# tinganchen/AlignQ

Hardware: AMD Instinct MI355X
Metric: images/sec (train step, CDF+ADMM) ResNet-20 8-bit (higher is better)
Workload: dtype f32; 1 GPU; resnet20 CIFAR-shape 3x32x32, 8W/8A CDF+ADMM full train step (cdf_alignment_admm/resnet-20-cifar-10), batch 128/GPU, HIP-graph replay, batch-norm folded into the site kernels, channels-last tensors, all Conv2d_Q convolutions on alignq_conv*_nhwc (exact-product bf16 MFMA); global_batch=128, parallelism=dp1

## Files before the change

alignq_amd/csrc/conv_kernels.hip:

```cpp
#include <hip/hip_runtime.h>
#include <stdint.h>
#include <stdlib.h>

#include "../../include/alignq.h"
#include "site_internal.h"
#include "wgrad_reduce_body.h"

namespace {

using namespace alignq_wgr;

typedef __bf16 bf16x8 __attribute__((ext_vector_type(8)));
typedef __bf16 bf16x4 __attribute__((ext_vector_type(4)));
typedef float f32x4 __attribute__((ext_vector_type(4)));
typedef short s16x4 __attribute__((ext_vector_type(4)));

__device__ __forceinline__ s16x4 tr_read(const __bf16* p) {
  return __builtin_amdgcn_ds_read_tr16_b64_v4i16((__attribute__((address_space(3))) s16x4*)(p));
}
__device__ __forceinline__ bf16x8 join8(s16x4 a, s16x4 b) {
  typedef short s16x8 __attribute__((ext_vector_type(8)));
  s16x8 v = {a[0], a[1], a[2], a[3], b[0], b[1], b[2], b[3]};
  return __builtin_bit_cast(bf16x8, v);
}


template <int xb>
__device__ __forceinline__ f32x4 fetch_act4(const float* __restrict__ x, int64_t off) {
  if constexpr (xb == 0) return *reinterpret_cast<const f32x4*>(x + off);
  if constexpr (xb == 2) {
    const s16x4 b = *reinterpret_cast<const s16x4*>(reinterpret_cast<const short*>(x) + off);
    return (f32x4){(float)b[0], (float)b[1], (float)b[2], (float)b[3]};
  }
  const char4 b = *reinterpret_cast<const char4*>(reinterpret_cast<const signed char*>(x) + off);
  return (f32x4){(float)b.x, (float)b.y, (float)b.z, (float)b.w};
}

struct BnLazy {
  const float* z;
  const float* ab;
  const float* save;
  const float* ktot;
  const float* part = nullptr;
  int n_tiles = 0, tile_f = 0;
  double inv_n = 1.0;
  float* dgamma = nullptr;
  float* dbeta = nullptr;
};

template <int C>
__device__ __forceinline__ void bn_totals_lds(const BnLazy& t, float* __restrict__ kt, bool publish) {
  static_assert(256 % C == 0, "thread -> (channel, group)");
  __shared__ double red[256][2];
  constexpr int G = 256 / C;
  const int tid = threadIdx.x;
  const int cp = C < t.tile_f ? C : t.tile_f;
  const int cyc = C / cp, cnt = t.n_tiles / cyc;
  const int c = tid % C, grp = tid / C;
// ... 597 lines not shown

template <int CIN, int COUT, int WDI, int KS, int PT>
__global__ __launch_bounds__(256) void dgrad_s2_kernel(const float* __restrict__ dy, const float* __restrict__ w,
                                                       float* __restrict__ dx, int H, int total_rows, float nlev,
                                                       const float* __restrict__ add, BnLazy lazy) {
  __shared__ __attribute__((aligned(16))) __bf16 lds[DgradS2Lds<CIN, COUT, WDI, KS, PT, false>::kBf16];
  dgrad_s2_body<CIN, COUT, WDI, KS, PT, false>(dy, w, dx, H, total_rows, nlev, add, lazy, lds, blockIdx.x);
}

template <int CIN, int COUT, int WDI, int KS, int PT>
int launch_dgrad_s2(const float* dy, const float* w, float* dx, int B, int H, float nlev, const float* add, BnLazy lazy,
                    hipStream_t st) {
  constexpr int TR = PT / WDI;
  static_assert(TR % 2 == 0, "even number of input rows per tile");
  if (H % TR) return ALIGNQ_EUNSUPPORTED;
  const int total_rows = B * H;
  hipLaunchKernelGGL((dgrad_s2_kernel<CIN, COUT, WDI, KS, PT>), total_rows / TR, 256, 0, st, dy, w, dx, H, total_rows, nlev,
                     add, lazy);
  hipError_t e = hipGetLastError();
  return e == hipSuccess ? 0 : (int)e;
}

constexpr int kStemPT = 128;
__device__ __forceinline__ void stem_stage(const float* __restrict__ x, int H, int row0, __bf16* Chi, __bf16* Cmi, __bf16* Clo) {
  const int tid = threadIdx.x;
  const int pix = tid >> 1, half = tid & 1;
  const int r = pix / 32, c = pix % 32;
  const int grow = row0 + r;
  const int ih = grow % H;
  float v[16];
#pragma unroll
  for (int j = 0; j < 16; j++) {
    const int k = 16 * half + j;
    const int tap = k / 3, ci = k % 3;
    const int ky = tap / 3, kx = tap % 3;
    const int yy = ih + ky - 1, xx = c + kx - 1;
    const bool ok = k < 27 && yy >= 0 && yy < H && xx >= 0 && xx < 32;
    v[j] = x[ok ? ((int64_t)(grow + ky - 1) * 32 + xx) * 3 + ci : 0];
    if (!ok) v[j] = 0.f;
  }
  bf16x8 h[2], m[2], l[2];
#pragma unroll
  for (int j = 0; j < 16; j++) {
    const __bf16 hi = (__bf16)v[j];
    const float r1 = v[j] - (float)hi;
    const __bf16 mi = (__bf16)r1;
    h[j >> 3][j & 7] = hi; m[j >> 3][j & 7] = mi; l[j >> 3][j & 7] = (__bf16)(r1 - (float)mi);
  }
  const int o = pix * 32 + 16 * half;
  *reinterpret_cast<bf16x8*>(Chi + o) = h[0]; *reinterpret_cast<bf16x8*>(Chi + o + 8) = h[1];
  *reinterpret_cast<bf16x8*>(Cmi + o) = m[0]; *reinterpret_cast<bf16x8*>(Cmi + o + 8) = m[1];
  *reinterpret_cast<bf16x8*>(Clo + o) = l[0]; *reinterpret_cast<bf16x8*>(Clo + o + 8) = l[1];
}

__global__ __launch_bounds__(256) void stem_fwd_kernel(const float* __restrict__ x, const float* __restrict__ w,
                                                       float* __restrict__ y, int H, int total_rows, float nlev,
                                                       float* __restrict__ bn_part) {
  __shared__ __attribute__((aligned(16))) __bf16 lds[3 * kStemPT * 32];
  __bf16* Chi = lds;
  __bf16* Cmi = lds + kStemPT * 32;
  __bf16* Clo = lds + 2 * kStemPT * 32;
  const int tid = threadIdx.x, lane = tid & 63, wv = tid >> 6;
  const int row0 = blockIdx.x * 4;
  stem_stage(x, H, row0, Chi, Cmi, Clo);
  const int m = lane & 15, q = lane >> 4;
  bf16x8 ab;
#pragma unroll
  for (int j = 0; j < 8; j++) {
    const int k = 8 * q + j;
    ab[j] = (__bf16)rintf((k < 27 ? w[m * 27 + k] : 0.f) * nlev);
  }
  __syncthreads();
  float bs[4] = {0.f, 0.f, 0.f, 0.f}, bq[4] = {0.f, 0.f, 0.f, 0.f};
  for (int g = wv; g < kStemPT / 16; g += 4) {
    const int p = g * 16 + (lane & 15);
// ... 18 lines not shown
      ROW_SHR_ADD(bs[e], 0x111); ROW_SHR_ADD(bs[e], 0x112); ROW_SHR_ADD(bs[e], 0x114); ROW_SHR_ADD(bs[e], 0x118);
      ROW_SHR_ADD(bq[e], 0x111); ROW_SHR_ADD(bq[e], 0x112); ROW_SHR_ADD(bq[e], 0x114); ROW_SHR_ADD(bq[e], 0x118);
    }
#undef ROW_SHR_ADD
    __syncthreads();
    if ((lane & 15) == 15) {
#pragma unroll
      for (int e = 0; e < 4; e++) {
        red[(wv * 16 + 4 * q + e) * 2] = bs[e];
        red[(wv * 16 + 4 * q + e) * 2 + 1] = bq[e];
      }
    }
    __syncthreads();
    if (tid < 16) {
      float s0 = 0.f, s1 = 0.f;
#pragma unroll
      for (int w2 = 0; w2 < 4; w2++) { s0 += red[(w2 * 16 + tid) * 2]; s1 += red[(w2 * 16 + tid) * 2 + 1]; }
      bn_part[((int64_t)tid * gridDim.x + blockIdx.x) * 2] = s0;
      bn_part[((int64_t)tid * gridDim.x + blockIdx.x) * 2 + 1] = s1;
    }
  }
}

__global__ __launch_bounds__(256) void stem_wgrad_kernel(const float* __restrict__ x, const float* __restrict__ dy,
                                                         float* __restrict__ slabs, int H, int n_tiles, BnLazy lazy) {
  __shared__ __attribute__((aligned(16))) __bf16 lds[3 * kStemPT * 32 + 3 * kStemPT * 16];
  __bf16* Ci[3] = {lds, lds + kStemPT * 32, lds + 2 * kStemPT * 32};
  __bf16* Di[3] = {lds + 3 * kStemPT * 32, lds + 3 * kStemPT * 32 + kStemPT * 16, lds + 3 * kStemPT * 32 + 2 * kStemPT * 16};
  const int tid = threadIdx.x, lane = tid & 63, wv = tid >> 6;
  const int g = lane >> 4, q = (lane & 15) >> 2, pcol = 4 * (lane & 3);
  f32x4 acc[2] = {{0.f, 0.f, 0.f, 0.f}, {0.f, 0.f, 0.f, 0.f}};
  __shared__ __attribute__((aligned(16))) float kt[32];
  if (lazy.z && lazy.part) bn_totals_lds<16>(lazy, kt, blockIdx.x == 0);
  for (int tile = blockIdx.x; tile < n_tiles; tile += gridDim.x) {
    const int row0 = tile * 4;
    f32x4 dvr[2], zvr[2];
#pragma unroll
    for (int it = 0; it < 2; it++) {
      const int i = tid + 256 * it;
      const int64_t off = ((int64_t)row0 * 32 + i / 4) * 16 + 4 * (tid % 4);
      dvr[it] = *reinterpret_cast<const f32x4*>(dy + off);
      zvr[it] = lazy.z ? *reinterpret_cast<const f32x4*>(lazy.z + off) : (f32x4){0.f, 0.f, 0.f, 0.f};
    }
    __syncthreads();
    stem_stage(x, H, row0, Ci[0], Ci[1], Ci[2]);
    {
      const int c4 = tid % 4;
      f32x4 la = {0, 0, 0, 0}, lm = la, li = la, lk0 = la, lk1 = la;
      if (lazy.z) {
        la = *reinterpret_cast<const f32x4*>(lazy.ab + 4 * c4);
        lm = *reinterpret_cast<const f32x4*>(lazy.save + 4 * c4);
        li = *reinterpret_cast<const f32x4*>(lazy.save + 16 + 4 * c4);
        const float* kp = lazy.part ? kt : lazy.ktot;
        lk0 = *reinterpret_cast<const f32x4*>(kp + 4 * c4);
        lk1 = *reinterpret_cast<const f32x4*>(kp + 16 + 4 * c4);
      }
#pragma unroll
      for (int it = 0; it < 2; it++) {
        const int i = tid + 256 * it;
        f32x4 dv = dvr[it];
        if (lazy.z) dv = la * (dv - lk0 - (zvr[it] - lm) * li * lk1);
        bf16x4 h4, m4, l4;
#pragma unroll
        for (int e = 0; e < 4; e++) {
          const __bf16 hi = (__bf16)dv[e];
          const float r1 = dv[e] - (float)hi;
          const __bf16 mi = (__bf16)r1;
          h4[e] = hi; m4[e] = mi; l4[e] = (__bf16)(r1 - (float)mi);
        }
        const int o = (i / 4) * 16 + 4 * c4;
        *reinterpret_cast<bf16x4*>(Di[0] + o) = h4;
        *reinterpret_cast<bf16x4*>(Di[1] + o) = m4;
        *reinterpret_cast<bf16x4*>(Di[2] + o) = l4;
      }
    }
    __syncthreads();
    {
      const int p0 = 32 * wv + 8 * g;
      bf16x8 a[3];
#pragma unroll
      for (int t = 0; t < 3; t++) {
        const __bf16* pa = Di[t] + (p0 + q) * 16 + pcol;
        a[t] = join8(tr_read(pa), tr_read(pa + 4 * 16));
      }
#pragma unroll
      for (int blk = 0; blk < 2; blk++) {
        bf16x8 b[3];
#pragma unroll
        for (int t = 0; t < 3; t++) {
          const __bf16* pb = Ci[t] + (p0 + q) * 32 + 16 * blk + pcol;
          b[t] = join8(tr_read(pb), tr_read(pb + 4 * 32));
        }
        f32x4 v = acc[blk];
        v = __builtin_amdgcn_mfma_f32_16x16x32_bf16(a[1], b[1], v, 0, 0, 0);
        v = __builtin_amdgcn_mfma_f32_16x16x32_bf16(a[0], b[2], v, 0, 0, 0);
        v = __builtin_amdgcn_mfma_f32_16x16x32_bf16(a[2], b[0], v, 0, 0, 0);
        v = __builtin_amdgcn_mfma_f32_16x16x32_bf16(a[0], b[1], v, 0, 0, 0);
        v = __builtin_amdgcn_mfma_f32_16x16x32_bf16(a[1], b[0], v, 0, 0, 0);
        v = __builtin_amdgcn_mfma_f32_16x16x32_bf16(a[0], b[0], v, 0, 0, 0);
        acc[blk] = v;
      }
    }
  }
  float* red = reinterpret_cast<float*>(lds);
  __syncthreads();
  if (wv > 0) {
#pragma unroll
    for (int blk = 0; blk < 2; blk++)
#pragma unroll
      for (int e = 0; e < 4; e++) red[(((wv - 1) * 2 + blk) * 4 + e) * 64 + lane] = acc[blk][e];
  }
  __syncthreads();
  if (wv == 0) {
    float* slab = slabs + (int64_t)blockIdx.x * (16 * 27);
#pragma unroll
    for (int blk = 0; blk < 2; blk++) {
#pragma unroll
      for (int e = 0; e < 4; e++) {
        float v = acc[blk][e];
#pragma unroll
        for (int w2 = 0; w2 < 3; w2++) v += red[((w2 * 2 + blk) * 4 + e) * 64 + lane];
        const int k = 16 * blk + (lane & 15), co = 4 * (lane >> 4) + e;
        if (k < 27) slab[co * 27 + k] = v;
// ... 10 lines not shown
  hipLaunchKernelGGL((convgen_fwd_kernel<CIN, COUT, WDI, KS, S, PT>), total_rows / TR, 256, 0, st, x, w, y, H, total_rows,
                     nlev, bn_part);
  hipError_t e = hipGetLastError();
  return e == hipSuccess ? 0 : (int)e;
}

template <int C, int WD, int PT>
int launch(const float* x, const float* w, float* y, int B, int H, int dgrad, float nlev, const float* add, float* bn_part,
           hipStream_t st, int xb = 0, float xlev = 1.0f) {
  constexpr int TR = PT / WD;
  const int total_rows = B * H;
  if (H % TR) return ALIGNQ_EUNSUPPORTED;
  const int grid = total_rows / TR;
  if (dgrad) hipLaunchKernelGGL((conv3x3_nhwc_kernel<C, WD, PT, true, 0>), grid, 256, 0, st, x, w, y, H, total_rows, nlev, add, nullptr, 1.0f);
  else if (xb == 2) hipLaunchKernelGGL((conv3x3_nhwc_kernel<C, WD, PT, false, 2>), grid, 256, 0, st, x, w, y, H, total_rows, nlev, add, bn_part, xlev);
  else if (xb == 1) hipLaunchKernelGGL((conv3x3_nhwc_kernel<C, WD, PT, false, 1>), grid, 256, 0, st, x, w, y, H, total_rows, nlev, add, bn_part, xlev);
  else hipLaunchKernelGGL((conv3x3_nhwc_kernel<C, WD, PT, false, 0>), grid, 256, 0, st, x, w, y, H, total_rows, nlev, add, bn_part, xlev);
  hipError_t e = hipGetLastError();
  return e == hipSuccess ? 0 : (int)e;
}

typedef float f32x16 __attribute__((ext_vector_type(16)));

template <int CIN, int COUT, int WDI, int KS, int S, int PT>
struct WgradGeo {
  static constexpr int WDO = WDI / S, TR = PT / WDO, NT = KS * KS;
  static constexpr int CB = (CIN < COUT ? CIN : COUT) >= 32 ? 32 : 16;
  static constexpr int XROWS = KS == 3 ? TR * S + (S == 1 ? 2 : 1) : TR;
  static constexpr int LW = KS == 3 ? WDI + 2 : WDO;
  static constexpr int XA = XROWS * LW * CB;
  static constexpr int DA = PT * CB;
  static constexpr int kRed = 3 * NT * 4 * 64 * 4;
  static constexpr int kBytes = (3 * (XA + DA) * 2) > kRed ? (3 * (XA + DA) * 2) : kRed;
  static constexpr int kFloats = kBytes / 4;
};
template <int C, int WD, int PT>
struct WgradLds : WgradGeo<C, C, WD, 3, 1, PT> {};

template <int CIN, int COUT, int WDI, int KS, int S, int PT, int XB = 0>
__device__ __forceinline__ void wgrad_body(const float* __restrict__ x, const float* __restrict__ dy,
                                           float* __restrict__ slabs, int H, int n_tiles, float* lds_f, int bx, int gx,
                                           int by, BnLazy lazy = BnLazy{nullptr, nullptr, nullptr, nullptr}, float xlev = 1.0f) {
  constexpr int xb = XB;
  using G = WgradGeo<CIN, COUT, WDI, KS, S, PT>;
  constexpr int WDO = G::WDO, TR = G::TR, NT = G::NT, CB = G::CB, LW = G::LW, XA = G::XA, DA = G::DA, XROWS = G::XROWS;
  constexpr int NBLK = CIN / CB;
  constexpr int NSTEP = PT / 32;
  static_assert(WDO % 8 == 0 && PT % 32 == 0, "a lane group's 8 pixels lie in one output row");
  __bf16* lds = reinterpret_cast<__bf16*>(lds_f);
  __bf16* Xi[3] = {lds, lds + XA, lds + 2 * XA};
  __bf16* Di[3] = {lds + 3 * XA, lds + 3 * XA + DA, lds + 3 * XA + 2 * DA};
  const int tid = threadIdx.x, lane = tid & 63, wv = tid >> 6;
  const int bi = by / NBLK, bj = by % NBLK;
  const int cob = CB == 32 ? (wv >> 1) : 0, cib = CB == 32 ? (wv & 1) : 0;
  const int g = lane >> 4, q = (lane & 15) >> 2, pcol = 4 * (lane & 3);

  f32x4 acc[NT];
#pragma unroll
  for (int t = 0; t < NT; t++) acc[t] = (f32x4){0.f, 0.f, 0.f, 0.f};

  constexpr int C4 = CB / 4;
  constexpr int N4 = XROWS * LW * C4;
  constexpr int M4 = PT * C4;
  constexpr int NIX = (N4 + 255) / 256, NID = (M4 + 255) / 256;
  f32x4 rx[NIX], rd[NID], rz[NID];
  const int per = (n_tiles + gx - 1) / gx;
  const int t_begin = bx * per, t_end = (t_begin + per < n_tiles) ? t_begin + per : n_tiles;
  int nxt = t_begin;
  if (nxt < t_end) {
    const int row0_ = nxt * TR;
    const int img_lo_ = (row0_ / H) * (H * S), img_hi_ = img_lo_ + H * S;
#pragma unroll
    for (int it = 0; it < NIX; it++) {
      const int i = tid + 256 * it;
      const int c4 = i % C4, col = (i / C4) % LW, lr = i / (C4 * LW);
      const int grow = KS == 3 ? row0_ * S - 1 + lr : (row0_ + lr) * S;
      const int gcol = KS == 3 ? col - 1 : col * S;
      const bool ok = i < N4 && gcol >= 0 && gcol < WDI && grow >= img_lo_ && grow < img_hi_;
      const int64_t off = ok ? ((int64_t)grow * WDI + gcol) * CIN + bj * CB + 4 * c4 : 0;
      rx[it] = fetch_act4<XB>(x, off);
      if (!ok) rx[it] = (f32x4){0.f, 0.f, 0.f, 0.f};
    }
#pragma unroll
    for (int it = 0; it < NID; it++) {
      const int i = tid + 256 * it;
      const int64_t off = i < M4 ? ((int64_t)row0_ * WDO + i / C4) * COUT + bi * CB + 4 * (i % C4) : 0;
      rd[it] = *reinterpret_cast<const f32x4*>(dy + off);
      if (lazy.z) rz[it] = *reinterpret_cast<const f32x4*>(lazy.z + off);
    }
  }
  f32x4 la = {0, 0, 0, 0}, lm = la, li = la, lk0 = la, lk1 = la;
  if (lazy.z) {
    const int cq = bi * CB + 4 * (tid % C4);
    la = *reinterpret_cast<const f32x4*>(lazy.ab + cq);
    lm = *reinterpret_cast<const f32x4*>(lazy.save + cq);
    li = *reinterpret_cast<const f32x4*>(lazy.save + COUT + cq);
    if (lazy.part) {
      __shared__ __attribute__((aligned(16))) float kt[2 * COUT];
      bn_totals_lds<COUT>(lazy, kt, false);
      lk0 = *reinterpret_cast<const f32x4*>(kt + cq);
      lk1 = *reinterpret_cast<const f32x4*>(kt + COUT + cq);
    } else {
      lk0 = *reinterpret_cast<const f32x4*>(lazy.ktot + cq);
      lk1 = *reinterpret_cast<const f32x4*>(lazy.ktot + COUT + cq);
    }
  }
  for (int tile = t_begin; tile < t_end; tile++) {
    __syncthreads();
#pragma unroll
    for (int it = 0; it < NIX; it++) {
      const int i = tid + 256 * it;
      if (i < N4) {
        const int c4 = i % C4, col = (i / C4) % LW, lr = i / (C4 * LW);
        bf16x4 h4, m4, l4;
#pragma unroll
        for (int e = 0; e < 4; e++) {
          const float v = rx[it][e];
          const __bf16 hi = (__bf16)v;
          const float r1 = v - (float)hi;
          const __bf16 mi = (__bf16)r1;
          h4[e] = hi; m4[e] = mi; l4[e] = (__bf16)(r1 - (float)mi);
        }
        const int o = (lr * LW + col) * CB + 4 * c4;
        *reinterpret_cast<bf16x4*>(Xi[0] + o) = h4;
        *reinterpret_cast<bf16x4*>(Xi[1] + o) = m4;
        *reinterpret_cast<bf16x4*>(Xi[2] + o) = l4;
      }
    }
#pragma unroll
    for (int it = 0; it < NID; it++) {
      const int i = tid + 256 * it;
      if (i < M4) {
        bf16x4 h4, m4, l4;
        f32x4 dv = rd[it];
        if (lazy.z) dv = la * (dv - lk0 - (rz[it] - lm) * li * lk1);
#pragma unroll
        for (int e = 0; e < 4; e++) {
          const float v = dv[e];
          const __bf16 hi = (__bf16)v;
          const float r1 = v - (float)hi;
          const __bf16 mi = (__bf16)r1;
          h4[e] = hi; m4[e] = mi; l4[e] = (__bf16)(r1 - (float)mi);
        }
        const int o = (i / C4) * CB + 4 * (i % C4);
        *reinterpret_cast<bf16x4*>(Di[0] + o) = h4;
        *reinterpret_cast<bf16x4*>(Di[1] + o) = m4;
        *reinterpret_cast<bf16x4*>(Di[2] + o) = l4;
      }
    }
    __syncthreads();
    nxt = tile + 1;
    if (nxt < t_end) {
      const int row0_ = nxt * TR;
      const int img_lo_ = (row0_ / H) * (H * S), img_hi_ = img_lo_ + H * S;
#pragma unroll
      for (int it = 0; it < NIX; it++) {
        const int i = tid + 256 * it;
        const int c4 = i % C4, col = (i / C4) % LW, lr = i / (C4 * LW);
        const int grow = KS == 3 ? row0_ * S - 1 + lr : (row0_ + lr) * S;
        const int gcol = KS == 3 ? col - 1 : col * S;
        const bool ok = i < N4 && gcol >= 0 && gcol < WDI && grow >= img_lo_ && grow < img_hi_;
        const int64_t off = ok ? ((int64_t)grow * WDI + gcol) * CIN + bj * CB + 4 * c4 : 0;
        rx[it] = fetch_act4<XB>(x, off);
        if (!ok) rx[it] = (f32x4){0.f, 0.f, 0.f, 0.f};
      }
#pragma unroll
      for (int it = 0; it < NID; it++) {
        const int i = tid + 256 * it;
        const int64_t off = i < M4 ? ((int64_t)row0_ * WDO + i / C4) * COUT + bi * CB + 4 * (i % C4) : 0;
        rd[it] = *reinterpret_cast<const f32x4*>(dy + off);
        if (lazy.z) rz[it] = *reinterpret_cast<const f32x4*>(lazy.z + off);
      }
    }
    for (int s = (CB == 16 ? wv : 0); s < NSTEP; s += (CB == 16 ? 4 : 1)) {
      const int p0 = 32 * s + 8 * g;
      const int r = p0 / WDO, c0 = p0 % WDO;
      bf16x8 a[3];
#pragma unroll
      for (int t = 0; t < 3; t++) {
        const __bf16* pa = Di[t] + (p0 + q) * CB + cob * 16 + pcol;
        a[t] = join8(tr_read(pa), tr_read(pa + 4 * CB));
      }
#pragma unroll
      for (int tap = 0; tap < NT; tap++) {
        const int ky = tap / KS, kx = tap % KS;
        bf16x8 b[3];
#pragma unroll
        for (int t = 0; t < 3; t++) {
          const __bf16* pb = Xi[t] + (KS == 3 ? ((r * S + ky) * LW + ((c0 + q) * S + kx)) : (r * LW + c0 + q)) * CB +
                             cib * 16 + pcol;
          b[t] = join8(tr_read(pb), tr_read(pb + 4 * (KS == 3 ? S : 1) * CB));
        }
        f32x4 v = acc[tap];
        v = __builtin_amdgcn_mfma_f32_16x16x32_bf16(a[1], b[1], v, 0, 0, 0);
        if (xb == 0) v = __builtin_amdgcn_mfma_f32_16x16x32_bf16(a[0], b[2], v, 0, 0, 0);
        v = __builtin_amdgcn_mfma_f32_16x16x32_bf16(a[2], b[0], v, 0, 0, 0);
        v = __builtin_amdgcn_mfma_f32_16x16x32_bf16(a[0], b[1], v, 0, 0, 0);
        v = __builtin_amdgcn_mfma_f32_16x16x32_bf16(a[1], b[0], v, 0, 0, 0);
        v = __builtin_amdgcn_mfma_f32_16x16x32_bf16(a[0], b[0], v, 0, 0, 0);
        acc[tap] = v;
      }
    }
  }
  float* slab = slabs + (int64_t)bx * (NT * CIN * COUT);
  if (xb != 0) {
    const float inv = 1.0f / xlev;
#pragma unroll
    for (int t = 0; t < NT; t++) acc[t] = acc[t] * inv;
  }
  if (CB == 16) {
    float* red = lds_f;
    __syncthreads();
    if (wv > 0) {
#pragma unroll
      for (int t = 0; t < NT; t++)
#pragma unroll
        for (int e = 0; e < 4; e++) red[(((wv - 1) * NT + t) * 4 + e) * 64 + lane] = acc[t][e];
    }
    __syncthreads();
    if (wv == 0) {
#pragma unroll
      for (int t = 0; t < NT; t++) {
#pragma unroll
        for (int e = 0; e < 4; e++) {
          float v = acc[t][e];
#pragma unroll
          for (int w2 = 0; w2 < 3; w2++) v += red[((w2 * NT + t) * 4 + e) * 64 + lane];
          __builtin_nontemporal_store(v, &slab[((int64_t)(bi * CB + 4 * (lane >> 4) + e) * NT + t) * CIN + bj * CB + (lane & 15)]);
        }
      }
    }
  } else {
#pragma unroll
    for (int t = 0; t < NT; t++)
#pragma unroll
      for (int e = 0; e < 4; e++)
        __builtin_nontemporal_store(acc[t][e], &slab[((int64_t)(bi * CB + cob * 16 + 4 * (lane >> 4) + e) * NT + t) * CIN + bj * CB + cib * 16 + (lane & 15)]);
  }
}

template <int C, int WD, int PT, int XB = 0>
__device__ __forceinline__ void wgrad3x3_body(const float* __restrict__ x, const float* __restrict__ dy,
                                              float* __restrict__ slabs, int H, int n_tiles, float* lds_f, int bx, int gx,
                                              int by, BnLazy lazy = BnLazy{nullptr, nullptr, nullptr, nullptr}, float xlev = 1.0f) {
  wgrad_body<C, C, WD, 3, 1, PT, XB>(x, dy, slabs, H, n_tiles, lds_f, bx, gx, by, lazy, xlev);
}

template <int CIN, int COUT, int WDI, int KS, int S, int PT>
__global__ __launch_bounds__(256) void wgradgen_kernel(const float* __restrict__ x, const float* __restrict__ dy,
                                                       float* __restrict__ slabs, int H, int n_tiles, BnLazy lazy) {
  __shared__ __attribute__((aligned(16))) float lds[WgradGeo<CIN, COUT, WDI, KS, S, PT>::kFloats];
  wgrad_body<CIN, COUT, WDI, KS, S, PT>(x, dy, slabs, H, n_tiles, lds, blockIdx.x, gridDim.x, blockIdx.y, lazy);
}

template <int C, int WD, int PT, int XB>
__global__ __launch_bounds__(256) void wgrad3x3_nhwc_kernel(const float* __restrict__ x, const float* __restrict__ dy,
                                                            float* __restrict__ slabs, int H, int n_tiles, float xlev) {
  __shared__ __attribute__((aligned(16))) float lds[WgradLds<C, WD, PT>::kFloats];
  wgrad3x3_body<C, WD, PT, XB>(x, dy, slabs, H, n_tiles, lds, blockIdx.x, gridDim.x, blockIdx.y,
                               BnLazy{nullptr, nullptr, nullptr, nullptr}, xlev);
}

template <int C, int WD, int PTD, int PTW, int XB>
__global__ __launch_bounds__(256) void conv3x3_bwd_kernel(const float* __restrict__ x, const float* __restrict__ dy,
                                                          const float* __restrict__ w, float* __restrict__ dx,
                                                          float* __restrict__ slabs, int H, int total_rows, float nlev,
                                                          int n_tiles_w, int splits, int nblk2,
                                                          const float* __restrict__ add, BnLazy lazy, float xlev, int dg_R,
                                                          RedFill fill, int n_dg) {
  constexpr int kBytesD = ConvLds<C, WD, PTD>::kBf16 * 2, kBytesW = WgradLds<C, WD, PTW>::kFloats * 4;
  static_assert(kBytesD >= 4096 || kBytesW >= 4096, "the filler role's 4 KB");
  __shared__ __attribute__((aligned(16))) unsigned char lds[kBytesD > kBytesW ? kBytesD : kBytesW];
  const int n_wg = splits * nblk2;
  if ((int)blockIdx.x < n_wg) {
    wgrad3x3_body<C, WD, PTW, XB>(x, dy, slabs, H, n_tiles_w, reinterpret_cast<float*>(lds), blockIdx.x % splits, splits,
                                  blockIdx.x / splits, lazy, xlev);
  } else if ((int)blockIdx.x >= n_wg + n_dg) {
    const int fb = blockIdx.x - n_wg - n_dg;
    int it = 0;
    while (it + 1 < kFill && fb >= fill.blk0[it + 1]) it++;
    wgrad_reduce_body<256>(fill.slabs[it], fill.n_slabs[it], fill.n_elem[it], fill.dw[it], fb - fill.blk0[it],
                           reinterpret_cast<float*>(lds));
  } else {
    int m = blockIdx.x - n_wg;
    if (dg_R > 0) {
      const int i = (m / (8 * dg_R)) * 8 + (m & 7), r = (m >> 3) % dg_R;
      m = dg_R * i + r;
    }
    conv3x3_body<C, WD, PTD, true>(dy, w, dx, H, total_rows, nlev, reinterpret_cast<__bf16*>(lds), m, add, nullptr, 0, lazy);
  }
}

template <int CIN, int COUT, int WDI, int PTW3, int PTW1, int PTD>
__global__ __launch_bounds__(256) void transition_bwd_kernel(const float* __restrict__ x, const float* __restrict__ dy3,
                                                             const float* __restrict__ dy1, const float* __restrict__ w3,
                                                             const float* __restrict__ w1, float* __restrict__ dx,
                                                             float* __restrict__ slabs3, float* __restrict__ slabs1, int Ho,
                                                             int n_tiles3, int n_tiles1, int splits3, int splits1, int n_d,
                                                             float nlev, const float* __restrict__ add, BnLazy lazy3,
                                                             BnLazy lazy1, int dg_R) {
  using G3 = WgradGeo<CIN, COUT, WDI, 3, 2, PTW3>;
  using G1 = WgradGeo<CIN, COUT, WDI, 1, 2, PTW1>;
  constexpr int NBY = (COUT / G3::CB) * (CIN / G3::CB);
  static_assert(G3::CB == G1::CB, "same channel blocking");
  constexpr int kD = DgradS2Lds<CIN, COUT, WDI, 3, PTD, true>::kBf16 * 2;
  constexpr int kW = G3::kBytes > G1::kBytes ? G3::kBytes : G1::kBytes;
  __shared__ __attribute__((aligned(16))) unsigned char lds[kD > kW ? kD : kW];
  const int n_w3 = splits3 * NBY;
  const int b = blockIdx.x;
  if (b < n_d) {
    int m = b;
    if (dg_R > 0) {
      const int i = (m / (8 * dg_R)) * 8 + (m & 7), r = (m >> 3) % dg_R;
      m = dg_R * i + r;
    }
    dgrad_s2_body<CIN, COUT, WDI, 3, PTD, true>(dy3, w3, dx, 2 * Ho, 0x7fffffff, nlev, add, lazy3,
                                                reinterpret_cast<__bf16*>(lds), m, dy1, w1, lazy1);
  } else if (b < n_d + n_w3) {
    const int c = b - n_d;
    wgrad_body<CIN, COUT, WDI, 3, 2, PTW3>(x, dy3, slabs3, Ho, n_tiles3, reinterpret_cast<float*>(lds), c % splits3, splits3,
                                           c / splits3, lazy3);
  } else {
    const int c = b - n_d - n_w3;
    wgrad_body<CIN, COUT, WDI, 1, 2, PTW1>(x, dy1, slabs1, Ho, n_tiles1, reinterpret_cast<float*>(lds), c % splits1, splits1,
                                           c / splits1, lazy1);
  }
}

__global__ __launch_bounds__(1024) void wgrad_reduce_kernel(const float* __restrict__ slabs, int n_slabs, int n_elem,
                                                            float* __restrict__ dw) {
  __shared__ __attribute__((aligned(16))) float part[4096];
  wgrad_reduce_body(slabs, n_slabs, n_elem, dw, blockIdx.x, part);
}

constexpr int kWgMulti = 32;
struct WgChunk {
  const float* slabs[kWgMulti];
  float* dw[kWgMulti];
  int n_slabs[kWgMulti];
  int n_elem[kWgMulti];
  int blk0[kWgMulti + 1];
};
__global__ __launch_bounds__(1024) void wgrad_reduce_multi_kernel(WgChunk c, int cnt) {
  __shared__ __attribute__((aligned(16))) float part[4096];
// ... 361 lines not shown

int alignq_conv_stem_bn_parts(int B, int H, int W) { return (W == 32 && B >= 1 && H >= 4 && H % 4 == 0) ? B * H / 4 : 0; }
int alignq_conv_stem_nhwc_fwd(const float* x, const float* wt, float* y, int B, int H, int W, int w_bit, float* bn_part,
                              void* stream) {
  if (!x || !wt || !y) return ALIGNQ_EINVAL;
  if (w_bit < 1 || w_bit > 8 || !alignq_conv_stem_bn_parts(B, H, W)) return ALIGNQ_EUNSUPPORTED;
  if (reinterpret_cast<uintptr_t>(y) & 15) return ALIGNQ_EUNSUPPORTED;
  hipLaunchKernelGGL(stem_fwd_kernel, B * H / 4, 256, 0, (hipStream_t)stream, x, wt, y, H, B * H, (float)((1 << w_bit) - 1),
                     bn_part);
  hipError_t e = hipGetLastError();
  return e == hipSuccess ? 0 : (int)e;
}
int alignq_conv_stem_nhwc_wgrad(const float* x, const float* dy, float* dw, void* ws, int B, int H, int W, int* n_slabs_out,
                                const float* bn_z, const float* bn_ab, const float* bn_save, const float* bn_ktot,
                                const float* bn_dx_part, float* bn_dgamma, float* bn_dbeta, void* stream) {
  if (!x || !dy || !ws || (!dw && !n_slabs_out)) return ALIGNQ_EINVAL;
  if (bn_z && (!bn_ab || !bn_save || (!bn_ktot && !bn_dx_part))) return ALIGNQ_EINVAL;
  if (!alignq_conv_stem_bn_parts(B, H, W) || (reinterpret_cast<uintptr_t>(dy) & 15)) return ALIGNQ_EUNSUPPORTED;
  hipStream_t st = (hipStream_t)stream;
  const int n_tiles = B * H / 4;
  const int splits = n_tiles < 256 ? n_tiles : 256;
  BnLazy lazy{bn_z, bn_ab, bn_save, bn_ktot};
  if (int rc = lazy_parts(lazy, bn_dx_part, bn_dgamma, bn_dbeta, B, 16, H * W)) return rc;
  hipLaunchKernelGGL(stem_wgrad_kernel, splits, 256, 0, st, x, dy, (float*)ws, H, n_tiles, lazy);
  hipError_t e = hipGetLastError();
  if (e != hipSuccess) return (int)e;
  if (n_slabs_out) { *n_slabs_out = splits; return 0; }
  hipLaunchKernelGGL(wgrad_reduce_kernel, wgrad_reduce_blocks(splits, 16 * 27), 1024, 0, st, (const float*)ws, splits, 16 * 27, dw);
  e = hipGetLastError();
  return e == hipSuccess ? 0 : (int)e;
}

}
```

Baseline: 126,800 images/sec.

## Prefetch multiple wgrad tiles into registers and drop unused low-part LDS plane

Weight-gradient kernels (stem, 16-channel 3x3 and stride-2 transition) now keep PF tiles of activations and output gradients in flight in registers, issuing the loads for tile t+PF right after parking tile t in LDS. This hides global-load latency behind the MFMA work in the small-channel layers, where each block does little compute per tile. Quantized (int8/int16) inputs are now kept raw in registers, with the zero padding tracked by a bitmask, and the third split plane for X is dropped from LDS because it is never used. The cost is much higher register pressure, which risks lower occupancy or spills.

New measurement: 126,500 images/sec. Within noise of the previous version (-0.3%).

```diff
diff --git a/alignq_amd/csrc/conv_kernels.hip b/alignq_amd/csrc/conv_kernels.hip
--- a/alignq_amd/csrc/conv_kernels.hip
+++ b/alignq_amd/csrc/conv_kernels.hip
@@ -34,6 +34,22 @@
   }
   const char4 b = *reinterpret_cast<const char4*>(reinterpret_cast<const signed char*>(x) + off);
   return (f32x4){(float)b.x, (float)b.y, (float)b.z, (float)b.w};
+}
+
+typedef signed char s8x4 __attribute__((ext_vector_type(4)));
+template <int xb> struct ActRaw { typedef f32x4 T; };
+template <> struct ActRaw<2> { typedef s16x4 T; };
+template <> struct ActRaw<1> { typedef s8x4 T; };
+template <int xb>
+__device__ __forceinline__ typename ActRaw<xb>::T fetch_act_raw(const float* __restrict__ x, int64_t off) {
+  if constexpr (xb == 0) return *reinterpret_cast<const f32x4*>(x + off);
+  if constexpr (xb == 2) return *reinterpret_cast<const s16x4*>(reinterpret_cast<const short*>(x) + off);
+  if constexpr (xb == 1) return *reinterpret_cast<const s8x4*>(reinterpret_cast<const signed char*>(x) + off);
+}
+template <int xb>
+__device__ __forceinline__ f32x4 act_raw_f32(typename ActRaw<xb>::T b) {
+  if constexpr (xb == 0) return b;
+  else return (f32x4){(float)b[0], (float)b[1], (float)b[2], (float)b[3]};
 }
 
 struct BnLazy {
@@ -677,13 +693,12 @@
 }
 
 constexpr int kStemPT = 128;
-__device__ __forceinline__ void stem_stage(const float* __restrict__ x, int H, int row0, __bf16* Chi, __bf16* Cmi, __bf16* Clo) {
+__device__ __forceinline__ void stem_fetch(const float* __restrict__ x, int H, int row0, float (&v)[16]) {
   const int tid = threadIdx.x;
   const int pix = tid >> 1, half = tid & 1;
   const int r = pix / 32, c = pix % 32;
   const int grow = row0 + r;
   const int ih = grow % H;
-  float v[16];
 #pragma unroll
   for (int j = 0; j < 16; j++) {
     const int k = 16 * half + j;
@@ -692,13 +707,20 @@
     const int yy = ih + ky - 1, xx = c + kx - 1;
     const bool ok = k < 27 && yy >= 0 && yy < H && xx >= 0 && xx < 32;
     v[j] = x[ok ? ((int64_t)(grow + ky - 1) * 32 + xx) * 3 + ci : 0];
-    if (!ok) v[j] = 0.f;
-  }
+  }
+}
+__device__ __forceinline__ void stem_park(const float (&v)[16], int H, int row0, __bf16* Chi, __bf16* Cmi, __bf16* Clo) {
+  const int tid = threadIdx.x;
+  const int pix = tid >> 1, half = tid & 1;
+  const int c = pix % 32, ih = (row0 + pix / 32) % H;
   bf16x8 h[2], m[2], l[2];
 #pragma unroll
   for (int j = 0; j < 16; j++) {
-    const __bf16 hi = (__bf16)v[j];
-    const float r1 = v[j] - (float)hi;
+    const int k = 16 * half + j;
+    const int yy = ih + (k / 3) / 3 - 1, xx = c + (k / 3) % 3 - 1;
+    const float vj = (k < 27 && yy >= 0 && yy < H && xx >= 0 && xx < 32) ? v[j] : 0.f;
+    const __bf16 hi = (__bf16)vj;
+    const float r1 = vj - (float)hi;
     const __bf16 mi = (__bf16)r1;
     h[j >> 3][j & 7] = hi; m[j >> 3][j & 7] = mi; l[j >> 3][j & 7] = (__bf16)(r1 - (float)mi);
   }
@@ -706,6 +728,11 @@
   *reinterpret_cast<bf16x8*>(Chi + o) = h[0]; *reinterpret_cast<bf16x8*>(Chi + o + 8) = h[1];
   *reinterpret_cast<bf16x8*>(Cmi + o) = m[0]; *reinterpret_cast<bf16x8*>(Cmi + o + 8) = m[1];
   *reinterpret_cast<bf16x8*>(Clo + o) = l[0]; *reinterpret_cast<bf16x8*>(Clo + o + 8) = l[1];
+}
+__device__ __forceinline__ void stem_stage(const float* __restrict__ x, int H, int row0, __bf16* Chi, __bf16* Cmi, __bf16* Clo) {
+  float v[16];
+  stem_fetch(x, H, row0, v);
+  stem_park(v, H, row0, Chi, Cmi, Clo);
 }
 
 __global__ __launch_bounds__(256) void stem_fwd_kernel(const float* __restrict__ x, const float* __restrict__ w,
@@ -770,6 +797,7 @@
   }
 }
 
+template <int PF>
 __global__ __launch_bounds__(256) void stem_wgrad_kernel(const float* __restrict__ x, const float* __restrict__ dy,
                                                          float* __restrict__ slabs, int H, int n_tiles, BnLazy lazy) {
   __shared__ __attribute__((aligned(16))) __bf16 lds[3 * kStemPT * 32 + 3 * kStemPT * 16];
@@ -779,35 +807,47 @@
   const int g = lane >> 4, q = (lane & 15) >> 2, pcol = 4 * (lane & 3);
   f32x4 acc[2] = {{0.f, 0.f, 0.f, 0.f}, {0.f, 0.f, 0.f, 0.f}};
   __shared__ __attribute__((aligned(16))) float kt[32];
-  if (lazy.z && lazy.part) bn_totals_lds<16>(lazy, kt, blockIdx.x == 0);
-  for (int tile = blockIdx.x; tile < n_tiles; tile += gridDim.x) {
-    const int row0 = tile * 4;
-    f32x4 dvr[2], zvr[2];
-#pragma unroll
-    for (int it = 0; it < 2; it++) {
-      const int i = tid + 256 * it;
-      const int64_t off = ((int64_t)row0 * 32 + i / 4) * 16 + 4 * (tid % 4);
-      dvr[it] = *reinterpret_cast<const f32x4*>(dy + off);
-      zvr[it] = lazy.z ? *reinterpret_cast<const f32x4*>(lazy.z + off) : (f32x4){0.f, 0.f, 0.f, 0.f};
-    }
-    __syncthreads();
-    stem_stage(x, H, row0, Ci[0], Ci[1], Ci[2]);
-    {
-      const int c4 = tid % 4;
-      f32x4 la = {0, 0, 0, 0}, lm = la, li = la, lk0 = la, lk1 = la;
-      if (lazy.z) {
-        la = *reinterpret_cast<const f32x4*>(lazy.ab + 4 * c4);
-        lm = *reinterpret_cast<const f32x4*>(lazy.save + 4 * c4);
-        li = *reinterpret_cast<const f32x4*>(lazy.save + 16 + 4 * c4);
-        const float* kp = lazy.part ? kt : lazy.ktot;
-        lk0 = *reinterpret_cast<const f32x4*>(kp + 4 * c4);
-        lk1 = *reinterpret_cast<const f32x4*>(kp + 16 + 4 * c4);
-      }
+  const int stride = gridDim.x;
+  float xr[PF][16];
+  f32x4 dvr[PF][2], zvr[PF][2];
+#pragma unroll
+  for (int st = 0; st < PF; st++) {
+    const int tile = blockIdx.x + st * stride;
+    if (tile < n_tiles) {
+      const int row0 = tile * 4;
 #pragma unroll
       for (int it = 0; it < 2; it++) {
         const int i = tid + 256 * it;
-        f32x4 dv = dvr[it];
-        if (lazy.z) dv = la * (dv - lk0 - (zvr[it] - lm) * li * lk1);
+        const int64_t off = ((int64_t)row0 * 32 + i / 4) * 16 + 4 * (tid % 4);
+        dvr[st][it] = *reinterpret_cast<const f32x4*>(dy + off);
+        if (lazy.z) zvr[st][it] = *reinterpret_cast<const f32x4*>(lazy.z + off);
+      }
+      stem_fetch(x, H, row0, xr[st]);
+    }
+  }
+  if (lazy.z && lazy.part) bn_totals_lds<16>(lazy, kt, blockIdx.x == 0);
+  const int c4 = tid % 4;
+  f32x4 la = {0, 0, 0, 0}, lm = la, li = la, lk0 = la, lk1 = la;
+  if (lazy.z) {
+    la = *reinterpret_cast<const f32x4*>(lazy.ab + 4 * c4);
+    lm = *reinterpret_cast<const f32x4*>(lazy.save + 4 * c4);
+    li = *reinterpret_cast<const f32x4*>(lazy.save + 16 + 4 * c4);
+    const float* kp = lazy.part ? kt : lazy.ktot;
+    lk0 = *reinterpret_cast<const f32x4*>(kp + 4 * c4);
+    lk1 = *reinterpret_cast<const f32x4*>(kp + 16 + 4 * c4);
+  }
+  for (int base = blockIdx.x; base < n_tiles; base += PF * stride) {
+#pragma unroll
+    for (int st = 0; st < PF; st++) {
+      const int tile = base + st * stride;
+      if (tile >= n_tiles) break;
+      __syncthreads();
+      stem_park(xr[st], H, tile * 4, Ci[0], Ci[1], Ci[2]);
+#pragma unroll
+      for (int it = 0; it < 2; it++) {
+        const int i = tid + 256 * it;
+        f32x4 dv = dvr[st][it];
+        if (lazy.z) dv = la * (dv - lk0 - (zvr[st][it] - lm) * li * lk1);
         bf16x4 h4, m4, l4;
 #pragma unroll
         for (int e = 0; e < 4; e++) {
@@ -821,32 +861,44 @@
         *reinterpret_cast<bf16x4*>(Di[1] + o) = m4;
         *reinterpret_cast<bf16x4*>(Di[2] + o) = l4;
       }
-    }
-    __syncthreads();
-    {
-      const int p0 = 32 * wv + 8 * g;
-      bf16x8 a[3];
-#pragma unroll
-      for (int t = 0; t < 3; t++) {
-        const __bf16* pa = Di[t] + (p0 + q) * 16 + pcol;
-        a[t] = join8(tr_read(pa), tr_read(pa + 4 * 16));
-      }
-#pragma unroll
-      for (int blk = 0; blk < 2; blk++) {
-        bf16x8 b[3];
+      __syncthreads();
+      const int nxt = tile + PF * stride;
+      if (nxt < n_tiles) {
+        const int row0 = nxt * 4;
+#pragma unroll
+        for (int it = 0; it < 2; it++) {
+          const int i = tid + 256 * it;
+          const int64_t off = ((int64_t)row0 * 32 + i / 4) * 16 + 4 * (tid % 4);
+          dvr[st][it] = *reinterpret_cast<const f32x4*>(dy + off);
+          if (lazy.z) zvr[st][it] = *reinterpret_cast<const f32x4*>(lazy.z + off);
+        }
+        stem_fetch(x, H, row0, xr[st]);
+      }
+      {
+        const int p0 = 32 * wv + 8 * g;
+        bf16x8 a[3];
 #pragma unroll
         for (int t = 0; t < 3; t++) {
-          const __bf16* pb = Ci[t] + (p0 + q) * 32 + 16 * blk + pcol;
-          b[t] = join8(tr_read(pb), tr_read(pb + 4 * 32));
+          const __bf16* pa = Di[t] + (p0 + q) * 16 + pcol;
+          a[t] = join8(tr_read(pa), tr_read(pa + 4 * 16));
         }
-        f32x4 v = acc[blk];
-        v = __builtin_amdgcn_mfma_f32_16x16x32_bf16(a[1], b[1], v, 0, 0, 0);
-        v = __builtin_amdgcn_mfma_f32_16x16x32_bf16(a[0], b[2], v, 0, 0, 0);
-        v = __builtin_amdgcn_mfma_f32_16x16x32_bf16(a[2], b[0], v, 0, 0, 0);
-        v = __builtin_amdgcn_mfma_f32_16x16x32_bf16(a[0], b[1], v, 0, 0, 0);
-        v = __builtin_amdgcn_mfma_f32_16x16x32_bf16(a[1], b[0], v, 0, 0, 0);
-        v = __builtin_amdgcn_mfma_f32_16x16x32_bf16(a[0], b[0], v, 0, 0, 0);
-        acc[blk] = v;
+#pragma unroll
+        for (int blk = 0; blk < 2; blk++) {
+          bf16x8 b[3];
+#pragma unroll
+          for (int t = 0; t < 3; t++) {
+            const __bf16* pb = Ci[t] + (p0 + q) * 32 + 16 * blk + pcol;
+            b[t] = join8(tr_read(pb), tr_read(pb + 4 * 32));
+          }
+          f32x4 v = acc[blk];
+          v = __builtin_amdgcn_mfma_f32_16x16x32_bf16(a[1], b[1], v, 0, 0, 0);
+          v = __builtin_amdgcn_mfma_f32_16x16x32_bf16(a[0], b[2], v, 0, 0, 0);
+          v = __builtin_amdgcn_mfma_f32_16x16x32_bf16(a[2], b[0], v, 0, 0, 0);
+          v = __builtin_amdgcn_mfma_f32_16x16x32_bf16(a[0], b[1], v, 0, 0, 0);
+          v = __builtin_amdgcn_mfma_f32_16x16x32_bf16(a[1], b[0], v, 0, 0, 0);
+          v = __builtin_amdgcn_mfma_f32_16x16x32_bf16(a[0], b[0], v, 0, 0, 0);
+          acc[blk] = v;
+        }
       }
     }
   }
@@ -903,7 +955,7 @@
 
 typedef float f32x16 __attribute__((ext_vector_type(16)));
 
-template <int CIN, int COUT, int WDI, int KS, int S, int PT>
+template <int CIN, int COUT, int WDI, int KS, int S, int PT, int NXP = 3>
 struct WgradGeo {
   static constexpr int WDO = WDI / S, TR = PT / WDO, NT = KS * KS;
   static constexpr int CB = (CIN < COUT ? CIN : COUT) >= 32 ? 32 : 16;
@@ -912,25 +964,27 @@
   static constexpr int XA = XROWS * LW * CB;
   static constexpr int DA = PT * CB;
   static constexpr int kRed = 3 * NT * 4 * 64 * 4;
-  static constexpr int kBytes = (3 * (XA + DA) * 2) > kRed ? (3 * (XA + DA) * 2) : kRed;
+  static constexpr int kImg = (NXP * XA + 3 * DA) * 2;
+  static constexpr int kBytes = kImg > kRed ? kImg : kRed;
   static constexpr int kFloats = kBytes / 4;
 };
-template <int C, int WD, int PT>
-struct WgradLds : WgradGeo<C, C, WD, 3, 1, PT> {};
-
-template <int CIN, int COUT, int WDI, int KS, int S, int PT, int XB = 0>
+template <int C, int WD, int PT, int XB = 0>
+struct WgradLds : WgradGeo<C, C, WD, 3, 1, PT, XB != 0 ? 2 : 3> {};
+
+template <int CIN, int COUT, int WDI, int KS, int S, int PT, int XB = 0, int PF = 1>
 __device__ __forceinline__ void wgrad_body(const float* __restrict__ x, const float* __restrict__ dy,
                                            float* __restrict__ slabs, int H, int n_tiles, float* lds_f, int bx, int gx,
                                            int by, BnLazy lazy = BnLazy{nullptr, nullptr, nullptr, nullptr}, float xlev = 1.0f) {
   constexpr int xb = XB;
-  using G = WgradGeo<CIN, COUT, WDI, KS, S, PT>;
+  constexpr int NXP = XB != 0 ? 2 : 3;
+  using G = WgradGeo<CIN, COUT, WDI, KS, S, PT, NXP>;
   constexpr int WDO = G::WDO, TR = G::TR, NT = G::NT, CB = G::CB, LW = G::LW, XA = G::XA, DA = G::DA, XROWS = G::XROWS;
   constexpr int NBLK = CIN / CB;
   constexpr int NSTEP = PT / 32;
   static_assert(WDO % 8 == 0 && PT % 32 == 0, "a lane group's 8 pixels lie in one output row");
   __bf16* lds = reinterpret_cast<__bf16*>(lds_f);
-  __bf16* Xi[3] = {lds, lds + XA, lds + 2 * XA};
-  __bf16* Di[3] = {lds + 3 * XA, lds + 3 * XA + DA, lds + 3 * XA + 2 * DA};
+  __bf16* Xi[3] = {lds, lds + XA, NXP == 3 ? lds + 2 * XA : nullptr};
+  __bf16* Di[3] = {lds + NXP * XA, lds + NXP * XA + DA, lds + NXP * XA + 2 * DA};
   const int tid = threadIdx.x, lane = tid & 63, wv = tid >> 6;
   const int bi = by / NBLK, bj = by % NBLK;
   const int cob = CB == 32 ? (wv >> 1) : 0, cib = CB == 32 ? (wv & 1) : 0;
@@ -944,30 +998,36 @@
   constexpr int N4 = XROWS * LW * C4;
   constexpr int M4 = PT * C4;
   constexpr int NIX = (N4 + 255) / 256, NID = (M4 + 255) / 256;
-  f32x4 rx[NIX], rd[NID], rz[NID];
+  typename ActRaw<XB>::T rx[PF][NIX];
+  f32x4 rd[PF][NID], rz[PF][NID];
+  unsigned xpad[PF];
   const int per = (n_tiles + gx - 1) / gx;
   const int t_begin = bx * per, t_end = (t_begin + per < n_tiles) ? t_begin + per : n_tiles;
-  int nxt = t_begin;
-  if (nxt < t_end) {
-    const int row0_ = nxt * TR;
-    const int img_lo_ = (row0_ / H) * (H * S), img_hi_ = img_lo_ + H * S;
-#pragma unroll
-    for (int it = 0; it < NIX; it++) {
-      const int i = tid + 256 * it;
-      const int c4 = i % C4, col = (i / C4) % LW, lr = i / (C4 * LW);
-      const int grow = KS == 3 ? row0_ * S - 1 + lr : (row0_ + lr) * S;
-      const int gcol = KS == 3 ? col - 1 : col * S;
-      const bool ok = i < N4 && gcol >= 0 && gcol < WDI && grow >= img_lo_ && grow < img_hi_;
-      const int64_t off = ok ? ((int64_t)grow * WDI + gcol) * CIN + bj * CB + 4 * c4 : 0;
-      rx[it] = fetch_act4<XB>(x, off);
-      if (!ok) rx[it] = (f32x4){0.f, 0.f, 0.f, 0.f};
-    }
-#pragma unroll
-    for (int it = 0; it < NID; it++) {
-      const int i = tid + 256 * it;
-      const int64_t off = i < M4 ? ((int64_t)row0_ * WDO + i / C4) * COUT + bi * CB + 4 * (i % C4) : 0;
-      rd[it] = *reinterpret_cast<const f32x4*>(dy + off);
-      if (lazy.z) rz[it] = *reinterpret_cast<const f32x4*>(lazy.z + off);
+#pragma unroll
+  for (int st = 0; st < PF; st++) {
+    const int nxt = t_begin + st;
+    if (nxt < t_end) {
+      const int row0_ = nxt * TR;
+      const int img_lo_ = (row0_ / H) * (H * S), img_hi_ = img_lo_ + H * S;
+      xpad[st] = 0;
+#pragma unroll
+      for (int it = 0; it < NIX; it++) {
+        const int i = tid + 256 * it;
+        const int c4 = i % C4, col = (i / C4) % LW, lr = i / (C4 * LW);
+        const int grow = KS == 3 ? row0_ * S - 1 + lr : (row0_ + lr) * S;
+        const int gcol = KS == 3 ? col - 1 : col * S;
+        const bool ok = i < N4 && gcol >= 0 && gcol < WDI && grow >= img_lo_ && grow < img_hi_;
+        const int64_t off = ok ? ((int64_t)grow * WDI + gcol) * CIN + bj * CB + 4 * c4 : 0;
+        rx[st][it] = fetch_act_raw<XB>(x, off);
+        if (!ok) xpad[st] |= 1u << it;
+      }
+#pragma unroll
+      for (int it = 0; it < NID; it++) {
+        const int i = tid + 256 * it;
+        const int64_t off = i < M4 ? ((int64_t)row0_ * WDO + i / C4) * COUT + bi * CB + 4 * (i % C4) : 0;
+        rd[st][it] = *reinterpret_cast<const f32x4*>(dy + off);
+        if (lazy.z) rz[st][it] = *reinterpret_cast<const f32x4*>(lazy.z + off);
+      }
     }
   }
   f32x4 la = {0, 0, 0, 0}, lm = la, li = la, lk0 = la, lk1 = la;
@@ -986,100 +1046,109 @@
       lk1 = *reinterpret_cast<const f32x4*>(lazy.ktot + COUT + cq);
     }
   }
-  for (int tile = t_begin; tile < t_end; tile++) {
-    __syncthreads();
-#pragma unroll
-    for (int it = 0; it < NIX; it++) {
-      const int i = tid + 256 * it;
-      if (i < N4) {
-        const int c4 = i % C4, col = (i / C4) % LW, lr = i / (C4 * LW);
-        bf16x4 h4, m4, l4;
-#pragma unroll
-        for (int e = 0; e < 4; e++) {
-          const float v = rx[it][e];
-          const __bf16 hi = (__bf16)v;
-          const float r1 = v - (float)hi;
-          const __bf16 mi = (__bf16)r1;
-          h4[e] = hi; m4[e] = mi; l4[e] = (__bf16)(r1 - (float)mi);
-        }
-        const int o = (lr * LW + col) * CB + 4 * c4;
-        *reinterpret_cast<bf16x4*>(Xi[0] + o) = h4;
-        *reinterpret_cast<bf16x4*>(Xi[1] + o) = m4;
-        *reinterpret_cast<bf16x4*>(Xi[2] + o) = l4;
-      }
-    }
-#pragma unroll
-    for (int it = 0; it < NID; it++) {
-      const int i = tid + 256 * it;
-      if (i < M4) {
-        bf16x4 h4, m4, l4;
-        f32x4 dv = rd[it];
-        if (lazy.z) dv = la * (dv - lk0 - (rz[it] - lm) * li * lk1);
-#pragma unroll
-        for (int e = 0; e < 4; e++) {
-          const float v = dv[e];
-          const __bf16 hi = (__bf16)v;
-          const float r1 = v - (float)hi;
-          const __bf16 mi = (__bf16)r1;
-          h4[e] = hi; m4[e] = mi; l4[e] = (__bf16)(r1 - (float)mi);
-        }
-        const int o = (i / C4) * CB + 4 * (i % C4);
-        *reinterpret_cast<bf16x4*>(Di[0] + o) = h4;
-        *reinterpret_cast<bf16x4*>(Di[1] + o) = m4;
-        *reinterpret_cast<bf16x4*>(Di[2] + o) = l4;
-      }
-    }
-    __syncthreads();
-    nxt = tile + 1;
-    if (nxt < t_end) {
-      const int row0_ = nxt * TR;
-      const int img_lo_ = (row0_ / H) * (H * S), img_hi_ = img_lo_ + H * S;
+  for (int base = t_begin; base < t_end; base += PF) {
+#pragma unroll
+    for (int st = 0; st < PF; st++) {
+      const int tile = base + st;
+      if (tile >= t_end) break;
+      __syncthreads();
 #pragma unroll
       for (int it = 0; it < NIX; it++) {
         const int i = tid + 256 * it;
-        const int c4 = i % C4, col = (i / C4) % LW, lr = i / (C4 * LW);
-        const int grow = KS == 3 ? row0_ * S - 1 + lr : (row0_ + lr) * S;
-        const int gcol = KS == 3 ? col - 1 : col * S;
-        const bool ok = i < N4 && gcol >= 0 && gcol < WDI && grow >= img_lo_ && grow < img_hi_;
-        const int64_t off = ok ? ((int64_t)grow * WDI + gcol) * CIN + bj * CB + 4 * c4 : 0;
-        rx[it] = fetch_act4<XB>(x, off);
-        if (!ok) rx[it] = (f32x4){0.f, 0.f, 0.f, 0.f};
+        if (i < N4) {
+          const int c4 = i % C4, col = (i / C4) % LW, lr = i / (C4 * LW);
+          f32x4 xv = act_raw_f32<XB>(rx[st][it]);
+          if ((xpad[st] >> it) & 1) xv = (f32x4){0.f, 0.f, 0.f, 0.f};
+          bf16x4 h4, m4, l4;
+#pragma unroll
+          for (int e = 0; e < 4; e++) {
+            const float v = xv[e];
+            const __bf16 hi = (__bf16)v;
+            const float r1 = v - (float)hi;
+            const __bf16 mi = (__bf16)r1;
+            h4[e] = hi; m4[e] = mi;
+            if constexpr (NXP == 3) l4[e] = (__bf16)(r1 - (float)mi);
+          }
+          const int o = (lr * LW + col) * CB + 4 * c4;
+          *reinterpret_cast<bf16x4*>(Xi[0] + o) = h4;
+          *reinterpret_cast<bf16x4*>(Xi[1] + o) = m4;
+          if constexpr (NXP == 3) *reinterpret_cast<bf16x4*>(Xi[2] + o) = l4;
+        }
       }
 #pragma unroll
       for (int it = 0; it < NID; it++) {
         const int i = tid + 256 * it;
-        const int64_t off = i < M4 ? ((int64_t)row0_ * WDO + i / C4) * COUT + bi * CB + 4 * (i % C4) : 0;
-        rd[it] = *reinterpret_cast<const f32x4*>(dy + off);
-        if (lazy.z) rz[it] = *reinterpret_cast<const f32x4*>(lazy.z + off);
-      }
-    }
-    for (int s = (CB == 16 ? wv : 0); s < NSTEP; s += (CB == 16 ? 4 : 1)) {
-      const int p0 = 32 * s + 8 * g;
-      const int r = p0 / WDO, c0 = p0 % WDO;
-      bf16x8 a[3];
-#pragma unroll
-      for (int t = 0; t < 3; t++) {
-        const __bf16* pa = Di[t] + (p0 + q) * CB + cob * 16 + pcol;
-        a[t] = join8(tr_read(pa), tr_read(pa + 4 * CB));
-      }
-#pragma unroll
-      for (int tap = 0; tap < NT; tap++) {
-        const int ky = tap / KS, kx = tap % KS;
-        bf16x8 b[3];
+        if (i < M4) {
+          bf16x4 h4, m4, l4;
+          f32x4 dv = rd[st][it];
+          if (lazy.z) dv = la * (dv - lk0 - (rz[st][it] - lm) * li * lk1);
+#pragma unroll
+          for (int e = 0; e < 4; e++) {
+            const float v = dv[e];
+            const __bf16 hi = (__bf16)v;
+            const float r1 = v - (float)hi;
+            const __bf16 mi = (__bf16)r1;
+            h4[e] = hi; m4[e] = mi; l4[e] = (__bf16)(r1 - (float)mi);
+          }
+          const int o = (i / C4) * CB + 4 * (i % C4);
+          *reinterpret_cast<bf16x4*>(Di[0] + o) = h4;
+          *reinterpret_cast<bf16x4*>(Di[1] + o) = m4;
+          *reinterpret_cast<bf16x4*>(Di[2] + o) = l4;
+        }
+      }
+      __syncthreads();
+      const int nxt = tile + PF;
+      if (nxt < t_end) {
+        const int row0_ = nxt * TR;
+        const int img_lo_ = (row0_ / H) * (H * S), img_hi_ = img_lo_ + H * S;
+        xpad[st] = 0;
+#pragma unroll
+        for (int it = 0; it < NIX; it++) {
+          const int i = tid + 256 * it;
+          const int c4 = i % C4, col = (i / C4) % LW, lr = i / (C4 * LW);
+          const int grow = KS == 3 ? row0_ * S - 1 + lr : (row0_ + lr) * S;
+          const int gcol = KS == 3 ? col - 1 : col * S;
+          const bool ok = i < N4 && gcol >= 0 && gcol < WDI && grow >= img_lo_ && grow < img_hi_;
+          const int64_t off = ok ? ((int64_t)grow * WDI + gcol) * CIN + bj * CB + 4 * c4 : 0;
+          rx[st][it] = fetch_act_raw<XB>(x, off);
+          if (!ok) xpad[st] |= 1u << it;
+        }
+#pragma unroll
+        for (int it = 0; it < NID; it++) {
+          const int i = tid + 256 * it;
+          const int64_t off = i < M4 ? ((int64_t)row0_ * WDO + i / C4) * COUT + bi * CB + 4 * (i % C4) : 0;
+          rd[st][it] = *reinterpret_cast<const f32x4*>(dy + off);
+          if (lazy.z) rz[st][it] = *reinterpret_cast<const f32x4*>(lazy.z + off);
+        }
+      }
+      for (int s = (CB == 16 ? wv : 0); s < NSTEP; s += (CB == 16 ? 4 : 1)) {
+        const int p0 = 32 * s + 8 * g;
+        const int r = p0 / WDO, c0 = p0 % WDO;
+        bf16x8 a[3];
 #pragma unroll
         for (int t = 0; t < 3; t++) {
-          const __bf16* pb = Xi[t] + (KS == 3 ? ((r * S + ky) * LW + ((c0 + q) * S + kx)) : (r * LW + c0 + q)) * CB +
-                             cib * 16 + pcol;
-          b[t] = join8(tr_read(pb), tr_read(pb + 4 * (KS == 3 ? S : 1) * CB));
+          const __bf16* pa = Di[t] + (p0 + q) * CB + cob * 16 + pcol;
+          a[t] = join8(tr_read(pa), tr_read(pa + 4 * CB));
         }
-        f32x4 v = acc[tap];
-        v = __builtin_amdgcn_mfma_f32_16x16x32_bf16(a[1], b[1], v, 0, 0, 0);
-        if (xb == 0) v = __builtin_amdgcn_mfma_f32_16x16x32_bf16(a[0], b[2], v, 0, 0, 0);
-        v = __builtin_amdgcn_mfma_f32_16x16x32_bf16(a[2], b[0], v, 0, 0, 0);
-        v = __builtin_amdgcn_mfma_f32_16x16x32_bf16(a[0], b[1], v, 0, 0, 0);
-        v = __builtin_amdgcn_mfma_f32_16x16x32_bf16(a[1], b[0], v, 0, 0, 0);
-        v = __builtin_amdgcn_mfma_f32_16x16x32_bf16(a[0], b[0], v, 0, 0, 0);
-        acc[tap] = v;
+#pragma unroll
+        for (int tap = 0; tap < NT; tap++) {
+          const int ky = tap / KS, kx = tap % KS;
+          bf16x8 b[NXP];
+#pragma unroll
+          for (int t = 0; t < NXP; t++) {
+            const __bf16* pb = Xi[t] + (KS == 3 ? ((r * S + ky) * LW + ((c0 + q) * S + kx)) : (r * LW + c0 + q)) * CB +
+                               cib * 16 + pcol;
+            b[t] = join8(tr_read(pb), tr_read(pb + 4 * (KS == 3 ? S : 1) * CB));
+          }
+          f32x4 v = acc[tap];
+          v = __builtin_amdgcn_mfma_f32_16x16x32_bf16(a[1], b[1], v, 0, 0, 0);
+          if constexpr (NXP == 3) v = __builtin_amdgcn_mfma_f32_16x16x32_bf16(a[0], b[2], v, 0, 0, 0);
+          v = __builtin_amdgcn_mfma_f32_16x16x32_bf16(a[2], b[0], v, 0, 0, 0);
+          v = __builtin_amdgcn_mfma_f32_16x16x32_bf16(a[0], b[1], v, 0, 0, 0);
+          v = __builtin_amdgcn_mfma_f32_16x16x32_bf16(a[1], b[0], v, 0, 0, 0);
+          v = __builtin_amdgcn_mfma_f32_16x16x32_bf16(a[0], b[0], v, 0, 0, 0);
+          acc[tap] = v;
+        }
       }
     }
   }
@@ -1120,11 +1189,11 @@
   }
 }
 
-template <int C, int WD, int PT, int XB = 0>
+template <int C, int WD, int PT, int XB = 0, int PF = 1>
 __device__ __forceinline__ void wgrad3x3_body(const float* __restrict__ x, const float* __restrict__ dy,
                                               float* __restrict__ slabs, int H, int n_tiles, float* lds_f, int bx, int gx,
                                               int by, BnLazy lazy = BnLazy{nullptr, nullptr, nullptr, nullptr}, float xlev = 1.0f) {
-  wgrad_body<C, C, WD, 3, 1, PT, XB>(x, dy, slabs, H, n_tiles, lds_f, bx, gx, by, lazy, xlev);
+  wgrad_body<C, C, WD, 3, 1, PT, XB, PF>(x, dy, slabs, H, n_tiles, lds_f, bx, gx, by, lazy, xlev);
 }
 
 template <int CIN, int COUT, int WDI, int KS, int S, int PT>
@@ -1137,7 +1206,7 @@
 template <int C, int WD, int PT, int XB>
 __global__ __launch_bounds__(256) void wgrad3x3_nhwc_kernel(const float* __restrict__ x, const float* __restrict__ dy,
                                                             float* __restrict__ slabs, int H, int n_tiles, float xlev) {
-  __shared__ __attribute__((aligned(16))) float lds[WgradLds<C, WD, PT>::kFloats];
+  __shared__ __attribute__((aligned(16))) float lds[WgradLds<C, WD, PT, XB>::kFloats];
   wgrad3x3_body<C, WD, PT, XB>(x, dy, slabs, H, n_tiles, lds, blockIdx.x, gridDim.x, blockIdx.y,
                                BnLazy{nullptr, nullptr, nullptr, nullptr}, xlev);
 }
@@ -1149,13 +1218,14 @@
                                                           int n_tiles_w, int splits, int nblk2,
                                                           const float* __restrict__ add, BnLazy lazy, float xlev, int dg_R,
                                                           RedFill fill, int n_dg) {
-  constexpr int kBytesD = ConvLds<C, WD, PTD>::kBf16 * 2, kBytesW = WgradLds<C, WD, PTW>::kFloats * 4;
+  constexpr int kBytesD = ConvLds<C, WD, PTD>::kBf16 * 2, kBytesW = WgradLds<C, WD, PTW, XB>::kFloats * 4;
+  constexpr int PF = C == 16 ? (XB == 2 ? 4 : 3) : 1;
   static_assert(kBytesD >= 4096 || kBytesW >= 4096, "the filler role's 4 KB");
   __shared__ __attribute__((aligned(16))) unsigned char lds[kBytesD > kBytesW ? kBytesD : kBytesW];
   const int n_wg = splits * nblk2;
   if ((int)blockIdx.x < n_wg) {
-    wgrad3x3_body<C, WD, PTW, XB>(x, dy, slabs, H, n_tiles_w, reinterpret_cast<float*>(lds), blockIdx.x % splits, splits,
-                                  blockIdx.x / splits, lazy, xlev);
+    wgrad3x3_body<C, WD, PTW, XB, PF>(x, dy, slabs, H, n_tiles_w, reinterpret_cast<float*>(lds), blockIdx.x % splits, splits,
+                                      blockIdx.x / splits, lazy, xlev);
   } else if ((int)blockIdx.x >= n_wg + n_dg) {
     const int fb = blockIdx.x - n_wg - n_dg;
     int it = 0;
@@ -1199,8 +1269,8 @@
                                                 reinterpret_cast<__bf16*>(lds), m, dy1, w1, lazy1);
   } else if (b < n_d + n_w3) {
     const int c = b - n_d;
-    wgrad_body<CIN, COUT, WDI, 3, 2, PTW3>(x, dy3, slabs3, Ho, n_tiles3, reinterpret_cast<float*>(lds), c % splits3, splits3,
-                                           c / splits3, lazy3);
+    wgrad_body<CIN, COUT, WDI, 3, 2, PTW3, 0, CIN == 16 ? 3 : 1>(x, dy3, slabs3, Ho, n_tiles3, reinterpret_cast<float*>(lds),
+                                                                 c % splits3, splits3, c / splits3, lazy3);
   } else {
     const int c = b - n_d - n_w3;
     wgrad_body<CIN, COUT, WDI, 1, 2, PTW1>(x, dy1, slabs1, Ho, n_tiles1, reinterpret_cast<float*>(lds), c % splits1, splits1,
@@ -1608,7 +1678,8 @@
   const int splits = n_tiles < 256 ? n_tiles : 256;
   BnLazy lazy{bn_z, bn_ab, bn_save, bn_ktot};
   if (int rc = lazy_parts(lazy, bn_dx_part, bn_dgamma, bn_dbeta, B, 16, H * W)) return rc;
-  hipLaunchKernelGGL(stem_wgrad_kernel, splits, 256, 0, st, x, dy, (float*)ws, H, n_tiles, lazy);
+  if (n_slabs_out) hipLaunchKernelGGL(stem_wgrad_kernel<4>, splits, 256, 0, st, x, dy, (float*)ws, H, n_tiles, lazy);
+  else hipLaunchKernelGGL(stem_wgrad_kernel<1>, splits, 256, 0, st, x, dy, (float*)ws, H, n_tiles, lazy);
   hipError_t e = hipGetLastError();
   if (e != hipSuccess) return (int)e;
   if (n_slabs_out) { *n_slabs_out = splits; return 0; }
```
